# khiner/MeshEditor

Measured on AMD Instinct MI355X. Metric: eigenpairs/sec (K/M assembly + 50-mode solve, 100k-tet mesh), higher is better.
Workload: dtype f64; 1 GPU; cube_s100k: Kuhn mesh 105456 tets / 446631 DOF, NumModes=50 NumFemModes=65, P=10 excitation points, one mesh per GPU; eigenpairs_per_mesh=65, kept_modes_per_mesh=50, parallelism=mesh-per-gpu x1

## Files before the change

mesheditor_amd/csrc/mh_api.hip:

```cpp
#include "mh_common.h"

#include <algorithm>
#include <cmath>
#include <memory>

namespace {
constexpr int TB = 256;

__global__ void k_export_blocks(const uint32_t *__restrict__ row_ptr, const uint32_t *__restrict__ col, const uint32_t *__restrict__ perm, uint32_t nnodes,
                                uint32_t *__restrict__ row_out, uint32_t *__restrict__ col_out) {
    const uint32_t r = blockIdx.x * blockDim.x + threadIdx.x;
    if (r >= nnodes) return;
    for (uint32_t p = row_ptr[r]; p < row_ptr[r + 1]; ++p) {
        row_out[p] = perm[r];
        col_out[p] = perm[col[p]];
    }
}
__global__ void k_ref_to_panel(const double *__restrict__ xref, const uint32_t *__restrict__ perm, uint32_t nnodes, uint32_t w, double *__restrict__ panel) {
    const size_t i = size_t(blockIdx.x) * blockDim.x + threadIdx.x;
    if (i >= size_t(nnodes) * 3 * w) return;
    const uint32_t c = uint32_t(i % w), comp = uint32_t((i / w) % 3), node = uint32_t(i / (size_t(3) * w));
    panel[i] = xref[size_t(c) * (size_t(3) * nnodes) + size_t(3) * perm[node] + comp];
}
template<typename S, typename D> __global__ void k_cast(const S *__restrict__ src, D *__restrict__ dst, size_t count) {
// ... 97 lines not shown
            size_t free_bytes = 0, total_bytes = 0;
            if (hipMemGetInfo(&free_bytes, &total_bytes) != hipSuccess) total_bytes = 0, (void)hipGetLastError();
            ctx->pool.set_cap_for_device(total_bytes);
        }
        HIP_CHECK(hipStreamCreateWithFlags(&ctx->stream, hipStreamNonBlocking));
        ROCBLAS_CHECK(rocblas_create_handle(&ctx->blas));
        ROCBLAS_CHECK(rocblas_set_stream(ctx->blas, ctx->stream));
        ROCBLAS_CHECK(rocblas_set_pointer_mode(ctx->blas, rocblas_pointer_mode_host));
        ROCBLAS_CHECK(rocblas_set_atomics_mode(ctx->blas, rocblas_atomics_not_allowed));
        *out = ctx;
        return MH_OK;
    } catch (const std::exception &e) {
        const int code = mh_guard(ctx, e);
        fprintf(stderr, "modalhip: %s\n", e.what());
        if (ctx->blas) rocblas_destroy_handle(ctx->blas);
        if (ctx->blas_aux) rocblas_destroy_handle(ctx->blas_aux);
        if (ctx->aux_stream) (void)hipStreamDestroy(ctx->aux_stream);
        if (ctx->aux2_stream) (void)hipStreamDestroy(ctx->aux2_stream);
        for (hipEvent_t ev : ctx->ahead_ev) (void)hipEventDestroy(ev);
        if (ctx->stream) (void)hipStreamDestroy(ctx->stream);
        delete ctx;
        return code;
    }
}
void mh_context_destroy(mh_context *ctx) {
    if (!ctx) return;
    (void)hipSetDevice(ctx->device);
    (void)hipStreamSynchronize(ctx->stream);
    if (ctx->blas) rocblas_destroy_handle(ctx->blas);
    if (ctx->blas_aux) rocblas_destroy_handle(ctx->blas_aux);
    if (ctx->aux_stream) (void)hipStreamDestroy(ctx->aux_stream);
    if (ctx->aux2_stream) (void)hipStreamDestroy(ctx->aux2_stream);
    for (hipEvent_t e : ctx->ahead_ev) (void)hipEventDestroy(e);
    if (ctx->stream) (void)hipStreamDestroy(ctx->stream);
    delete ctx;
}
const char *mh_last_error(const mh_context *ctx) { return ctx ? ctx->last_error.c_str() : "null context"; }
int mh_context_synchronize(mh_context *ctx) {
    if (!ctx) return MH_EINVAL;
    try {
        HIP_CHECK(hipStreamSynchronize(ctx->stream));
        return MH_OK;
    } catch (const std::exception &e) { return mh_guard(ctx, e); }
}
void *mh_context_stream(mh_context *ctx) { return ctx ? ctx->stream : nullptr; }
int mh_context_time_kernels(mh_context *ctx, int enable) {
    if (!ctx) return MH_EINVAL;
    try {
        mh_timer_flush(ctx);
        ctx->time_kernels = enable != 0;
        for (auto &t : ctx->totals) t = {};
        return MH_OK;
    } catch (const std::exception &e) { return mh_guard(ctx, e); }
}
int mh_context_kernel_class_stats(mh_context *ctx, int kernel_class, uint64_t *launches, double *total_ms, double *total_work) {
    if (!ctx || kernel_class < 0 || kernel_class >= MH_KERNEL_CLASSES) return MH_EINVAL;
    try {
        mh_timer_flush(ctx);
        const auto &t = ctx->totals[kernel_class];
        if (launches) *launches = t.launches;
        if (total_ms) *total_ms = t.ms;
        if (total_work) *total_work = t.work;
        return MH_OK;
    } catch (const std::exception &e) { return mh_guard(ctx, e); }
}
int mh_context_kernel_stats(mh_context *ctx, uint64_t *launches, double *total_ms, double *total_bytes) {
// ... 200 lines not shown
```

mesheditor_amd/csrc/mh_common.h:

```cpp
#pragma once
#include "../../include/modalhip.h"

#include <hip/hip_runtime.h>
#include <rocblas/rocblas.h>
#include <rocsolver/rocsolver.h>

#include <algorithm>
#include <cstdarg>
#include <cstdio>
#include <cstdlib>
#include <cstring>
#include <iterator>
#include <map>
#include <mutex>
#include <stdexcept>
#include <string>
#include <vector>

struct MhError : std::runtime_error {
    int code;
    MhError(int c, const std::string &m) : std::runtime_error(m), code(c) {}
};

[[noreturn]] inline void mh_throw(int code, const char *fmt, ...) {
// ... 206 lines not shown
            else if (rocblas_set_stream(blas_aux, aux_stream) != rocblas_status_success) {
                (void)rocblas_destroy_handle(blas_aux);
                blas_aux = nullptr;
            }
        }
        return aux_stream != nullptr && blas_aux != nullptr;
    }
    hipStream_t aux2_stream{nullptr};
    std::vector<hipEvent_t> ahead_ev;
    bool aux2_stream_ready(size_t events = 0) {
        if (!aux2_stream && hipStreamCreateWithFlags(&aux2_stream, hipStreamNonBlocking) != hipSuccess) aux2_stream = nullptr, (void)hipGetLastError();
        while (aux2_stream && ahead_ev.size() < events) {
            hipEvent_t e = nullptr;
            if (hipEventCreateWithFlags(&e, hipEventDisableTiming) != hipSuccess) { (void)hipGetLastError(); return false; }
            ahead_ev.push_back(e);
        }
        return aux2_stream != nullptr;
    }
    rocblas_handle blas{nullptr};
    rocblas_handle blas_aux{nullptr};
    DevicePool pool;
    std::string last_error;
    hipEvent_t ev0{nullptr}, ev1{nullptr};
    void *gram_ws{nullptr};
    size_t gram_ws_bytes{0};
    uint32_t *iota{nullptr};
    unsigned long long *sytrd_xch{nullptr};
    uint32_t sytrd_epoch{0};
    int *sytrd_flag{nullptr};
    unsigned long long *sytrd_xch_wide{nullptr};
    uint32_t sytrd_epoch_wide{0};
    bool exchange_disabled{false};
    uint32_t sytrd_redos{0};
    unsigned long long *rr_check{nullptr};
    bool time_kernels{false};
    std::vector<std::pair<hipEvent_t, hipEvent_t>> timer_events;
    std::vector<double> timer_work;
    std::vector<int> timer_class;
    size_t timer_used{0};
    struct ClassTotals {
        double ms{0}, work{0};
        uint64_t launches{0};
    } totals[MH_KERNEL_CLASSES];
};
void mh_timer_flush(mh_context *ctx);
struct TimedLaunch {
    mh_context *ctx;
    bool on;
    size_t slot{0};
    TimedLaunch(mh_context *c, int kernel_class, double work) : ctx(c), on(c->time_kernels) {
        if (!on) return;
        if (ctx->timer_used == ctx->timer_events.size()) {
            hipEvent_t a, b;
            HIP_CHECK(hipEventCreate(&a));
            HIP_CHECK(hipEventCreate(&b));
            ctx->timer_events.emplace_back(a, b);
            ctx->timer_work.push_back(0);
            ctx->timer_class.push_back(0);
        }
        slot = ctx->timer_used++;
        ctx->timer_work[slot] = work;
        ctx->timer_class[slot] = kernel_class;
        HIP_CHECK(hipEventRecord(ctx->timer_events[slot].first, ctx->stream));
    }
    ~TimedLaunch() {
        if (on) (void)hipEventRecord(ctx->timer_events[slot].second, ctx->stream);
// ... 152 lines not shown
    } catch (const std::exception &e) {                \
        return mh_guard(ctx_guard_, e);                \
    }

inline unsigned div_up(size_t a, size_t b) { return unsigned((a + b - 1) / b); }

void mh_phase_shared_lock(int device);
void mh_phase_shared_unlock(int device);
struct MhSharedPhase {
    const int device;
    explicit MhSharedPhase(int dev) : device(dev) { mh_phase_shared_lock(device); }
    ~MhSharedPhase() { mh_phase_shared_unlock(device); }
    MhSharedPhase(const MhSharedPhase &) = delete;
    MhSharedPhase &operator=(const MhSharedPhase &) = delete;
};
std::mutex &mh_solve_mutex();
void mh_build_system(mh_context *ctx, const mh_mesh *mesh, const mh_material &mat, mh_system *sys);
void mh_build_hierarchy(mh_system *sys, double sigma, bool defer = false);
void mh_finish_hierarchy(mh_system *sys);
uint32_t mh_shift_invert_panel(mh_system *sys, double sigma, const double *b, double *x, uint32_t w, double rel_tol, uint32_t max_iters, double *worst_rel);
uint32_t mh_graph_aggregates(const std::vector<uint32_t> &row_ptr, const std::vector<uint32_t> &col, uint32_t n, uint32_t target, uint32_t max_order, std::vector<uint32_t> &agg_of);
void mh_select_patches(mh_system *sys, float threshold);
void mh_build_patch_inverses(mh_context *ctx, const BsrLevel &lvl, PatchSet &ps);
template<typename T>
void mh_apply_patches(mh_context *ctx, const PatchSet &ps, const T *in, const T *minus, uint32_t w, T coef, T *d, T *x, double *z, uint32_t wz, T *scratch);
void mh_gram(mh_context *ctx, size_t n, const double *x, uint32_t wa, const double *y, uint32_t wb, double *g, uint32_t ld, uint32_t ldy = 0, const uint32_t *ymap = nullptr);
void mh_combine(mh_context *ctx, size_t n, const double *x, uint32_t wx, const double *w, uint32_t ww, const double *p, uint32_t wp, const double *ct, uint32_t nc,
                double *out1, uint32_t n1, double *out2, bool accumulate = false, uint32_t ldx = 0, const uint32_t *xmap = nullptr, uint32_t ld1 = 0,
                const uint32_t *omap = nullptr, uint32_t col_begin = 0, uint32_t col_count = 0);
bool mh_tridiag_lowest_wide(mh_context *ctx, const double *d, const double *e, uint32_t m, uint32_t k, double *w, double *z, uint32_t ldz, double *work, int *info2,
                            double *quality_host);
void mh_apply_q(mh_context *ctx, const double *a, const double *tau, uint32_t m, double *z, uint32_t ldz, uint32_t ncols);
bool mh_tridiag_lowest(mh_context *ctx, const double *d, const double *e, uint32_t m, uint32_t k, double *w, double *z, uint32_t ldz, double *ufac,
                       double *quality, double *lam_scratch);
void mh_spd_inverse_small(mh_context *ctx, const double *a, uint32_t lda, uint32_t w, double *out, uint32_t ldo, int *info);
void mh_potrf(mh_context *ctx, double *a, uint32_t ld, uint32_t w, int *info);
void mh_potrf_small(mh_context *ctx, double *a, uint32_t w, int *info);
void mh_potrf_small_inverse(mh_context *ctx, double *a, uint32_t w, int *info, const double *dscale, double *linv);
bool mh_sytrd_gave_up(mh_context *ctx);
void mh_sytrd_wide(mh_context *ctx, double *a, uint32_t m, double *d, double *e, double *tau);
void mh_sytrd_small(mh_context *ctx, double *a, uint32_t m, double *d, double *e, double *tau, int variant = -1);
void mh_small_gemm(mh_context *ctx, bool ta, bool tb, uint32_t M, uint32_t N, uint32_t K, double alpha, const double *a, uint32_t lda, const double *b, uint32_t ldb, double beta, double *c,
                   uint32_t ldc);
void mh_short_product(mh_context *ctx, size_t n, const double *a, uint32_t m, const double *ct, uint32_t nc, double *out, double *partial, uint32_t slices);
void mh_pack_stacked(mh_context *ctx, const double *c1, uint32_t r1, const double *c2, uint32_t r2, uint32_t cols, double scale, double *ct);
void mh_pack_coefficients(mh_context *ctx, const double *c1, uint32_t n1, const double *c2, uint32_t n2, uint32_t m, uint32_t ld, double *ct);
void mh_spmm_mapped(mh_context *ctx, const BsrLevel &lvl, const double *vals9, const double *x, double *y, const double *mscal, double *y2, uint32_t w, uint32_t ldy,
                    uint32_t wreal, const uint32_t *omap, const double *res_theta = nullptr, double *res_out = nullptr, double *res_partial = nullptr,
                    const double *res_dinv = nullptr);
bool mh_spmm_f32_cheb_step(mh_context *ctx, const BsrLevel &lvl, const float *d_in, float *d_out, float *r, float *x, const float *dinv, float c1, float c2,
                           uint32_t w);
void mh_spmm_f32(mh_context *ctx, const BsrLevel &lvl, const float *x, float *y, uint32_t w);
void mh_spmm_mixed(mh_context *ctx, const BsrLevel &lvl, const float *x, double *y, uint32_t w);
const uint32_t *mh_identity_map(mh_context *ctx);
void mh_spmm(mh_context *ctx, const BsrLevel &lvl, const double *vals9, const double *x, double *y, const double *mscal, double *y2, uint32_t w);
```

mesheditor_amd/csrc/mh_dense.hip:

```cpp
#include "mh_common.h"

#include <optional>

#include <map>

struct PerDeviceOnce {
    static constexpr int MaxDevices = 64;
    std::once_flag flag[MaxDevices];
    template<typename F> void run(int device, F &&f) { std::call_once(flag[device >= 0 && device < MaxDevices ? device : 0], std::forward<F>(f)); }
};

static bool mh_test_own_gemm() {
    static const bool on = getenv("MH_TEST") && strstr(getenv("MH_TEST"), "own_gemm");
    return on;
}
namespace {
constexpr int KC = 32;

typedef double double4_t __attribute__((ext_vector_type(4)));

__host__ __device__ inline int pad_pitch(int w) {
    int p = ((w + 15) / 16) * 16;
    if ((p % 32) != 16) p += 16;
    return p;
// ... 1445 lines not shown
    for (int i = 0; i < m; ++i) X[size_t(i) * k + j] *= sc;
}
__global__ void __launch_bounds__(256) k_tridiag_residual(const double *__restrict__ D, const double *__restrict__ E, int m, const double *__restrict__ lam, const double *__restrict__ Z, int ldz,
                                                         unsigned long long *__restrict__ quality) {
    __shared__ double d[WIDE_T], e[WIDE_T], red[32], worst_of[4];
    const int tid = threadIdx.x, j = blockIdx.x;
    for (int i = tid; i < m; i += 256) d[i] = D[i], e[i] = i + 1 < m ? E[i] : 0.0;
    __syncthreads();
    double tnorm, pivmin;
    tridiag_scale(d, e, m, tid, 256, red, tnorm, pivmin);
    const double *z = Z + size_t(j) * ldz, lj = lam[j];
    double worst = 0.0;
    bool bad = false;
    for (int i = tid; i < m; i += 256) {
        const double r = (d[i] - lj) * z[i] + (i ? e[i - 1] * z[i - 1] : 0.0) + (i + 1 < m ? e[i] * z[i + 1] : 0.0);
        bad |= !(fabs(r) <= 1.7976931348623157e308);
        worst = fmax(worst, fabs(r));
    }
    if (bad) worst = __longlong_as_double(0x7ff8000000000000ll);
    for (int off = 32; off > 0; off >>= 1) {
        const double o = __shfl_xor(worst, off, 64);
        worst = (o != o || worst != worst) ? __longlong_as_double(0x7ff8000000000000ll) : fmax(worst, o);
    }
    if ((tid & 63) == 0) worst_of[tid >> 6] = worst;
    __syncthreads();
    if (tid == 0) {
        double q = 0.0;
        bool nan = false;
        for (int a = 0; a < 4; ++a) nan |= worst_of[a] != worst_of[a], q = fmax(q, worst_of[a]);
        q = nan ? __longlong_as_double(0x7ff8000000000000ll) : q / fmax(tnorm, 2.2250738585072014e-308);
        atomicMax(quality, static_cast<unsigned long long>(__double_as_longlong(q)));
    }
}
__global__ void __launch_bounds__(1024) k_tridiag_lowest(const double *__restrict__ D, const double *__restrict__ E, int m, int k, double *__restrict__ w,
                                                        double *__restrict__ z, int ldz, double *__restrict__ ufac, double *__restrict__ quality, const double *__restrict__ lam_in) {
    extern __shared__ __attribute__((aligned(16))) double sm[];
    double *d = sm, *e = d + 256, *e2 = e + 256, *lam = e2 + 256, *lo = lam + 256, *hi = lo + 256, *coef = hi + 256, *red = coef + 256;
    int *cnt = reinterpret_cast<int *>(red + 1024);
    double *X = red + 1024 + 512;
    const int tid = threadIdx.x, lane = tid & 63;
    if (tid < 256) {
        d[tid] = tid < m ? D[tid] : 0.0;
        const double ev = tid + 1 < m ? E[tid] : 0.0;
        e[tid] = ev;
        e2[tid] = ev * ev;
    }
    __syncthreads();
    {
        double gl = 1.7976931348623157e308, gh = -1.7976931348623157e308;
        for (int i = tid; i < m; i += 1024) {
            const double r = (i ? fabs(e[i - 1]) : 0.0) + fabs(e[i]);
            gl = fmin(gl, d[i] - r);
            gh = fmax(gh, d[i] + r);
        }
        for (int off = 32; off > 0; off >>= 1) {
            gl = fmin(gl, __shfl_xor(gl, off, 64));
            gh = fmax(gh, __shfl_xor(gh, off, 64));
        }
        if (lane == 0) { red[tid >> 6] = gl; red[16 + (tid >> 6)] = gh; }
    }
    __syncthreads();
    double glo = red[0], ghi = red[16];
    for (int q = 1; q < 16; ++q) { glo = fmin(glo, red[q]); ghi = fmax(ghi, red[16 + q]); }
    const double tnorm = fmax(fabs(glo), fabs(ghi));
    const double eps = 2.220446049250313e-16;
    double e2max = 0;
    for (int i = 0; i < m; ++i) e2max = fmax(e2max, e2[i]);
    const double pivmin = 2.2250738585072014e-308 * fmax(1.0, e2max);
// ... 156 lines not shown
            }
            __syncthreads();
            left = wave_sum_lds(red, m, lane);
            if (left > 0.5 || j == 0) break;
        }
        if ((tid >> 3) == j) my_inv2 = 1.0 / left;
        if (tid == 0) lo[j] = 1.0 / sqrt(left);
    }
    __syncthreads();
    for (int idx = tid; idx < m * k; idx += 1024) X[idx] *= lo[idx % k];
    __syncthreads();
    const long long t_gs = wall_clock64();
    double worst = 0;
    for (int idx = tid; idx < m * k; idx += 1024) {
        const int i = idx / k, j = idx % k;
        const double x = X[idx];
        const double r = (d[i] - lam[j]) * x + (i ? e[i - 1] * X[idx - k] : 0.0) + (i + 1 < m ? e[i] * X[idx + k] : 0.0);
        worst = fmax(worst, fabs(r));
        z[size_t(j) * ldz + i] = x;
    }
    for (int off = 32; off > 0; off >>= 1) worst = fmax(worst, __shfl_xor(worst, off, 64));
    __syncthreads();
    if (lane == 0) red[tid >> 6] = worst;
    __syncthreads();
    if (tid == 0) {
        double q = 0;
        for (int a = 0; a < 16; ++a) q = fmax(q, red[a]);
        *quality = q / fmax(tnorm, 2.2250738585072014e-308);
        quality[1] = double(t_bisect - t_start);
        quality[2] = double(t_invit - t_bisect);
        quality[3] = double(t_gs - t_invit);
        quality[4] = double(wall_clock64() - t_gs);
    }
    if (tid < k) w[tid] = lam[tid];
}
}

bool mh_tridiag_lowest(mh_context *ctx, const double *d, const double *e, uint32_t m, uint32_t k, double *w, double *z, uint32_t ldz, double *ufac, double *quality,
                       double *lam_scratch) {
    if (m < 2 || m > 256 || k < 1 || k > m || k > 128) return false;
    const size_t lds = (size_t(7) * 256 + 1024 + 512 + size_t(m) * k) * sizeof(double);
    if (lds > 158 * 1024) return false;
    static PerDeviceOnce attr;
    attr.run(ctx->device, [] { HIP_CHECK(hipFuncSetAttribute(reinterpret_cast<const void *>(&k_tridiag_lowest), hipFuncAttributeMaxDynamicSharedMemorySize, 160 * 1024)); });
    constexpr bool spread = true;
    if (spread) {
        k_tridiag_values<1><<<k, 256, 0, ctx->stream>>>(d, e, int(m), lam_scratch);
        KERNEL_CHECK();
    }
    k_tridiag_lowest<<<1, 1024, lds, ctx->stream>>>(d, e, int(m), int(k), w, z, int(ldz), ufac, quality, spread ? lam_scratch : nullptr);
    KERNEL_CHECK();
    return true;
}

bool mh_tridiag_lowest_wide(mh_context *ctx, const double *d, const double *e, uint32_t m, uint32_t k, double *w, double *z, uint32_t ldz, double *work, int *info2, double *quality_host) {
    if (m <= 256 || m > WIDE_T || k < 1 || k > 256 || k > m) return false;
    const size_t km = size_t(k) * m;
    double *xt = work, *xt2 = xt + km, *ufac = xt2 + km, *g = ufac + 3 * km, *linv = g + size_t(k) * k, *qual = linv + size_t(k) * k;
    k_tridiag_values<3><<<k, 256, 0, ctx->stream>>>(d, e, int(m), w);
    KERNEL_CHECK();
    k_tridiag_invit<<<div_up(k, 64), 64, 0, ctx->stream>>>(d, e, int(m), int(k), w, xt, ufac);
    KERNEL_CHECK();
    DevArray<int> info4_array(ctx, 4);
    int *info4 = info4_array.get();
    HIP_CHECK(hipMemsetAsync(info4, 0, 4 * sizeof(int), ctx->stream));
    for (int pass = 0; pass < 2; ++pass) {
        const double *src = pass == 0 ? xt : xt2;
        mh_small_gemm(ctx, false, true, k, k, m, 1.0, src, k, src, k, 0.0, g, k);
        mh_potrf(ctx, g, k, k, info4 + 2 * pass);
        HIP_CHECK(hipMemsetAsync(linv, 0, size_t(k) * k * sizeof(double), ctx->stream));
        ROCBLAS_CHECK(rocblas_dtrtri(ctx->blas, rocblas_fill_lower, rocblas_diagonal_non_unit, rocblas_int(k), g, rocblas_int(k), linv, rocblas_int(k)));
        if (pass == 0) mh_small_gemm(ctx, false, false, k, m, k, 1.0, linv, k, src, k, 0.0, xt2, k);
        else mh_small_gemm(ctx, true, true, m, k, k, 1.0, src, k, linv, k, 0.0, z, ldz);
    }
    HIP_CHECK(hipMemsetAsync(qual, 0, sizeof(double), ctx->stream));
    k_tridiag_residual<<<k, 256, 0, ctx->stream>>>(d, e, int(m), w, z, int(ldz), reinterpret_cast<unsigned long long *>(qual));
    KERNEL_CHECK();
    int hinfo[4] = {0, 0, 0, 0};
    HIP_CHECK(hipMemcpyAsync(quality_host, qual, sizeof(double), hipMemcpyDeviceToHost, ctx->stream));
    HIP_CHECK(hipMemcpyAsync(hinfo, info4, sizeof(hinfo), hipMemcpyDeviceToHost, ctx->stream));
    HIP_CHECK(hipStreamSynchronize(ctx->stream));
    if (hinfo[0] != 0 || hinfo[2] != 0) *quality_host = std::numeric_limits<double>::quiet_NaN();
    return true;
// ... 403 lines not shown
```

mesheditor_amd/csrc/mh_eigs.hip:

```cpp
#include "mh_common.h"

#include <algorithm>
#include <cmath>
#include <memory>
#include <condition_variable>
#include <mutex>
#include <numeric>
#include <optional>
#include <type_traits>

__global__ void k_shift_values(const double *kval, const double *mval, size_t nblocks, double sigma, double *aval);
__global__ void k_diag_inverse(const uint32_t *row_ptr, const uint32_t *col, const double *aval, uint32_t nnodes, double *dinv);
__global__ void k_coarse_matrix(const uint32_t *row_ptr, const uint32_t *col, const double *aval, const double *tmat, const uint32_t *agg_of, const uint32_t *agg_ptr,
                                const uint32_t *agg_nodes, uint32_t nagg, double *a0);
__global__ void k_fix_coarse_diag(double *a0, uint32_t n0, double rel);

namespace {
constexpr int TB = 256;

std::mutex g_solve_mutex;
struct Switches {
    bool verbose = getenv("MH_VERBOSE") != nullptr;
    bool fp32_prec = !(getenv("MH_PRECOND_FP64") && atoi(getenv("MH_PRECOND_FP64")) != 0);
    int deg2 = 0, deg1 = 0, gamma = 0;
    double cheb_ratio = 0.0, cheb_ratio1 = 0.0;
    bool test_sytrd_giveup = getenv("MH_TEST") && strstr(getenv("MH_TEST"), "sytrd_giveup");
    bool no_tridiag_wide = getenv("MH_TEST") && strstr(getenv("MH_TEST"), "no_tridiag_wide");
    bool test_last_resort = getenv("MH_TEST") && strstr(getenv("MH_TEST"), "last_resort");
    bool test_coarse_pivot = getenv("MH_TEST") && strstr(getenv("MH_TEST"), "coarse_pivot");
    bool test_selfcheck_fail = getenv("MH_TEST") && strstr(getenv("MH_TEST"), "selfcheck_fail");
    bool lmax_low = getenv("MH_TEST") && strstr(getenv("MH_TEST"), "lmax_low");
    bool potrf_chain = getenv("MH_TEST") && strstr(getenv("MH_TEST"), "potrf_chain");
    bool no_poly_start = getenv("MH_TEST") && strstr(getenv("MH_TEST"), "no_poly_start");
    Switches() {
        if (const char *c = getenv("MH_CYCLE")) {
            double v[5] = {0, 0, 0, 0, 0};
            sscanf(c, "%lf,%lf,%lf,%lf,%lf", &v[0], &v[1], &v[2], &v[3], &v[4]);
            deg2 = std::max(0, int(v[0])), deg1 = std::max(0, int(v[1])), gamma = std::max(0, int(v[2]));
            cheb_ratio = v[3];
            cheb_ratio1 = v[4];
        }
    }
};
const Switches &switches() {
    static const Switches s;
    return s;
}
constexpr int kPowerIterations = 20;
constexpr uint32_t kPrecondColumns = 256;
constexpr uint32_t kSkipP = 4;
constexpr uint32_t kGuardPercent = 10;
constexpr float kFlatShape = 1e-4f;
constexpr size_t kDenseLastResort = 12288;
constexpr int kLastResortCg = 8;

struct PhaseLock {
    std::mutex m;
    std::condition_variable cv;
    int readers = 0, writers_waiting = 0;
    bool writer = false;
    void lock_shared() {
        std::unique_lock<std::mutex> l(m);
        cv.wait(l, [&] { return !writer && writers_waiting == 0; });
        ++readers;
    }
    void unlock_shared() {
// ... 529 lines not shown
        rmax = fmax(rmax, fabs(r)), azmax = fmax(azmax, abs_az), zmax = fmax(zmax, fabs(zs[i]));
    }
    red[0][tid] = nan ? INFINITY : rmax, red[1][tid] = azmax, red[2][tid] = zmax;
    __syncthreads();
    for (int h = 128; h > 0; h >>= 1) {
        if (tid < uint32_t(h))
            for (int q = 0; q < 3; ++q) red[q][tid] = fmax(red[q][tid], red[q][tid + h]);
        __syncthreads();
    }
    if (tid == 0) {
        const double rel = red[0][0] / fmax(red[1][0] + fabs(th) * red[2][0], 1e-300);
        atomicMax(worst, (unsigned long long)__double_as_longlong(rel == rel ? rel : INFINITY));
    }
}
void rr_selfcheck(mh_context *ctx, const double *saved, uint32_t m, const double *z, uint32_t ldz, const double *theta, uint32_t ncols) {
    if (!ncols) return;
    if (!ctx->rr_check) {
        ctx->rr_check = static_cast<unsigned long long *>(ctx->pool.alloc(256));
        HIP_CHECK(hipMemsetAsync(ctx->rr_check, 0, 256, ctx->stream));
    }
    k_rr_selfcheck<<<3, 256, 0, ctx->stream>>>(saved, m, z, ldz, theta, ncols, ctx->rr_check);
    KERNEL_CHECK();
}

int host_info(DevArray<int> &info) { int hinfo = 0; info.download(&hinfo, 1); return hinfo; }
bool sytrd_gave_up(mh_context *ctx, int flag, double *gA, const double *saved, uint32_t m) {
    if (!flag && !switches().test_sytrd_giveup) return false;
    ++ctx->sytrd_redos;
    HIP_CHECK(hipMemcpyAsync(gA, saved, size_t(m) * m * sizeof(double), hipMemcpyDeviceToDevice, ctx->stream));
    return true;
}
bool accept_partial(mh_context *ctx, double quality, double *evals, const double *lam, uint32_t nwant) {
    if (!(quality < 1e-10)) return false;
    HIP_CHECK(hipMemcpyAsync(evals, lam, size_t(nwant) * sizeof(double), hipMemcpyDeviceToDevice, ctx->stream));
    return true;
}

int eig_tridiag_small(mh_context *ctx, double *gA, uint32_t m, double *evals, double *ework, DevArray<int> &info, uint32_t nwant, std::vector<double> *host_evals) {
    DevArray<double> z(ctx, size_t(m) * m), tau(ctx, m);
    const bool partial = nwant && nwant < m;
    DevArray<double> zl(ctx, partial ? size_t(m) * nwant : 0);
    double *zres = z.get();
    uint32_t ncols = m;
    HIP_CHECK(hipMemcpyAsync(z.get(), gA, size_t(m) * m * sizeof(double), hipMemcpyDeviceToDevice, ctx->stream));
    for (int attempt = 0; attempt < 2; ++attempt) {
        mh_sytrd_small(ctx, gA, m, evals, ework, tau, attempt == 0 ? -1 : 0);
        int gave_up = 0;
        const bool flagged = attempt == 0 && ctx->sytrd_flag;
        if (flagged) HIP_CHECK(hipMemcpyAsync(&gave_up, ctx->sytrd_flag, sizeof(int), hipMemcpyDeviceToHost, ctx->stream));
        if (partial) {
            DevArray<double> wv(ctx, 2 * m + 8), ufac(ctx, size_t(3) * m * nwant);
            double *zout = attempt == 0 ? zl.get() : z.get();
            if (mh_tridiag_lowest(ctx, evals, ework, m, nwant, wv, zout, m, ufac, wv.get() + m, wv.get() + m + 8)) {
                double qv[5] = {1, 0, 0, 0, 0};
                std::vector<double> lam_host(host_evals ? nwant : 0);
                HIP_CHECK(hipMemcpyAsync(qv, wv.get() + m, sizeof(qv), hipMemcpyDeviceToHost, ctx->stream));
                if (host_evals) HIP_CHECK(hipMemcpyAsync(lam_host.data(), wv.get(), size_t(nwant) * sizeof(double), hipMemcpyDeviceToHost, ctx->stream));
                HIP_CHECK(hipStreamSynchronize(ctx->stream));
                if (flagged && sytrd_gave_up(ctx, gave_up, gA, z, m)) continue;
                if (switches().verbose)
                    fprintf(stderr, "[rr] tridiagonal m %u lowest %u: residual / ||T|| %.2e; us: multisection %.0f, inverse iteration %.0f, Gram-Schmidt %.0f, output %.0f\n", m,
                            nwant, qv[0], qv[1] * 0.01, qv[2] * 0.01, qv[3] * 0.01, qv[4] * 0.01);
                if (accept_partial(ctx, qv[0], evals, wv, nwant)) {
                    if (host_evals) host_evals->swap(lam_host);
                    zres = zout, ncols = nwant;
                    break;
                }
            }
        }
        if (flagged) {
            HIP_CHECK(hipStreamSynchronize(ctx->stream));
            if (sytrd_gave_up(ctx, gave_up, gA, z, m)) continue;
        }
        ROCBLAS_CHECK(rocsolver_dstedc(ctx->blas, rocblas_evect_tridiagonal, m, evals, ework, z, m, info));
        if (const int hinfo = host_info(info)) return hinfo;
        break;
    }
    mh_apply_q(ctx, gA, tau, m, zres, m, ncols);
    if (zres == zl.get()) rr_selfcheck(ctx, z.get(), m, zres, m, evals, ncols);
    HIP_CHECK(hipMemcpyAsync(gA, zres, size_t(m) * ncols * sizeof(double), hipMemcpyDeviceToDevice, ctx->stream));
    return 0;
}

std::optional<int> eig_tridiag_wide(mh_context *ctx, double *gA, uint32_t m, double *evals, double *ework, DevArray<int> &info, uint32_t nwant) {
    DevArray<double> z(ctx, size_t(m) * m), saved(ctx, size_t(m) * m), tau(ctx, m);
    HIP_CHECK(hipMemcpyAsync(saved.get(), gA, size_t(m) * m * sizeof(double), hipMemcpyDeviceToDevice, ctx->stream));
    mh_sytrd_wide(ctx, gA, m, evals, ework, tau);
    int gave_up = 0;
    HIP_CHECK(hipMemcpyAsync(&gave_up, ctx->sytrd_flag, sizeof(int), hipMemcpyDeviceToHost, ctx->stream));
    HIP_CHECK(hipStreamSynchronize(ctx->stream));
    if (sytrd_gave_up(ctx, gave_up, gA, saved, m)) return std::nullopt;
    if (nwant && nwant < m && nwant <= 256 && !switches().no_tridiag_wide) {
        DevArray<double> work(ctx, size_t(5) * nwant * m + size_t(2) * nwant * nwant + 8), lam(ctx, nwant);
        double quality = 1.0;
        if (mh_tridiag_lowest_wide(ctx, evals, ework, m, nwant, lam, z, m, work, info, &quality)) {
            if (switches().verbose) fprintf(stderr, "[rr] tridiagonal m %u lowest %u (wide): residual / ||T|| %.2e\n", m, nwant, quality);
            if (accept_partial(ctx, quality, evals, lam, nwant)) {
                mh_apply_q(ctx, gA, tau, m, z, m, nwant);
                rr_selfcheck(ctx, saved.get(), m, z, m, evals, nwant);
                HIP_CHECK(hipMemcpyAsync(gA, z.get(), size_t(m) * nwant * sizeof(double), hipMemcpyDeviceToDevice, ctx->stream));
                HIP_CHECK(hipStreamSynchronize(ctx->stream));
                return 0;
            }
        }
    }
    ROCBLAS_CHECK(rocsolver_dstedc(ctx->blas, rocblas_evect_tridiagonal, m, evals, ework, z, m, info));
    if (const int hinfo = host_info(info)) return hinfo;
    ROCBLAS_CHECK(rocsolver_dormtr(ctx->blas, rocblas_side_left, rocblas_fill_lower, rocblas_operation_none, m, m, gA, m, tau, z, m));
    HIP_CHECK(hipMemcpyAsync(gA, z.get(), size_t(m) * m * sizeof(double), hipMemcpyDeviceToDevice, ctx->stream));
    HIP_CHECK(hipStreamSynchronize(ctx->stream));
    return 0;
// ... 515 lines not shown
            mh_spmm(ctx, sys->L2, sys->L2.aval, p, ap, nullptr, nullptr, w);
            dot(p, ap, pap, w);
            k_cg_advance<<<grid1(n * w), TB, 0, st>>>(z, rr, p, ap, rz, pap, n * w, w);
            KERNEL_CHECK();
            if (k + 1 == iters) break;
            prec.apply(rr, zz, w);
            dot(rr, zz, rz_new, w);
            k_cg_direction<<<grid1(n * w), TB, 0, st>>>(p, zz, rz_new, rz, n * w, w);
            KERNEL_CHECK();
            HIP_CHECK(hipMemcpyAsync(rz.get(), rz_new.get(), w * sizeof(double), hipMemcpyDeviceToDevice, st));
        }
    }
};
}

namespace {
struct BlockLobpcg {
    mh_system *sys;
    mh_context *ctx;
    hipStream_t st;
    const size_t n;
    const uint32_t nev, b, mmax;
    const double sigma, residual_tol;
    const uint32_t max_iters;
    const float *seed_basis;
    const uint32_t seed_rows, seed_cols;
    const volatile unsigned char *cancel;
    volatile float *progress;
    mh_profile &prof;
    mh_profile *profile;
    SharedPhase iterating;
    Timer t_iter;
    double precond_seconds = 0;
    double best_worst_active = 1e300;
    int floor_strikes = 0;
    std::vector<double> hist_active;
    uint32_t pairs_at_floor = 0;
    DevArray<double> X, AX, MX, Xn, AXn, MXn, W, AW, MW, P, MP, Pn, MPn, R, Rw;
    DevArray<double> gA, gM, gM0, gA0, App, evals, ework, Cp, T1, H, H2, G, dscale, Linv, theta_d, rn_d, mn_d, scratch, Ct, norms_d, theta_act_d, Hp, Up, Vp, T1p;
    DevArray<double> Linv_p, T1p2;
    DevArray<uint32_t> idx_d, pos_d;
    DevArray<double> Rr, res_partial, res_blocks, res_norms_d;
    std::vector<double> rr_evals;
    std::vector<uint32_t> res_act, res_pos;
    std::vector<double> res_norms;
    uint32_t res_pitch = 0;
    bool res_ready = false, rw_from_rr = false;
    DevArray<int> info;
    int inner_cg = 0;
    std::unique_ptr<Precond<float>> prec32;
    std::unique_ptr<Precond<double>> prec64;
    std::unique_ptr<PanelCg> panel_cg;
    const bool verbose = switches().verbose, fp32_prec = switches().fp32_prec;
    const bool pproj_ok;
    const bool scaled_norms;
    bool warm = false;
    bool w_implicit = false;
    int last_spread = 1 << 20;
    bool p_needs_explicit = false;
    uint32_t wp = 0;
    uint32_t iters = 0, nconv = 0, redos_at_start = 0;
    bool poly_allowed = true;
    std::vector<double> theta, rn, mn, xn, norms, theta_act, hist_worst;
    double anorm = 0;
    std::vector<uint32_t> act, order, hist_nconv;
    std::vector<uint8_t> locked;
// ... 301 lines not shown
                mh_throw(MH_ENOTCONVERGED, "LOBPCG: %u of %u pairs converged; the others sit at the rounding floor (residual %.1e and growing, best %.1e, tolerance %.1e)", nconv, nev,
                         worst_active, best_worst_active, residual_tol);
        }
        return false;
    }

    void search_directions(uint32_t it) {
        w = uint32_t(act.size());
        idx_d.upload(act.data(), w);
        const double *residuals = Rw.get();
        if (rw_from_rr) {
            if (act == res_act && res_pitch == w) {
                residuals = Rr.get();
            } else {
                std::vector<uint32_t> &pos = res_pos;
                pos.assign(w, 0);
                size_t q = 0;
                for (uint32_t k = 0; k < w; ++k) {
                    while (q < res_act.size() && res_act[q] != act[k]) ++q;
                    if (q == res_act.size()) mh_throw(MH_EHIP, "active column %u was not active before", act[k]);
                    pos[k] = uint32_t(q);
                }
                pos_d.upload(pos.data(), w);
                k_gather_cols<<<grid1(n * w), TB, 0, st>>>(Rr, pos_d, Rw, n, res_pitch, w);
                KERNEL_CHECK();
            }
        } else {
            k_gather_cols<<<grid1(n * w), TB, 0, st>>>(R, idx_d, Rw, n, b, w);
            KERNEL_CHECK();
        }
        for (uint32_t k = 0; k < w; ++k) theta_act[k] = theta[act[k]];
        theta_act_d.upload(theta_act.data(), w);
        {
            Timer tp(ctx);
            precondition(residuals, W, w);
            precond_seconds += tp.stop();
            prof.op_applications += w;
        }
        bool ok = true;
        p_implicit = false;
        if (pproj_ok && wp) {
            gram(ctx, n, MX, b, W, w, H, b);
            mh_pack_stacked(ctx, H, b, nullptr, 0, w, -1.0, Ct);
            mh_combine(ctx, n, X, b, nullptr, 0, nullptr, 0, Ct, w, W, w, nullptr, true);
            mh_spmm(ctx, sys->L2, sys->L2.aval, W, AW, sys->L2.mval, MW, w);
            gram(ctx, n, P, wp, MW, w, Hp, wp);
            lazy_images = true;
            w_implicit = false;
            ok = chol_orthonormalise(W, MW, AW, w, false, true, Hp, wp);
            if (!ok) mh_throw(MH_ENOTCONVERGED, "search directions lost rank at iteration %u", it);
            if (p_needs_explicit) {
                mh_pack_stacked(ctx, Hp, wp, nullptr, 0, w, -1.0, Ct);
                mh_combine(ctx, n, P, wp, nullptr, 0, nullptr, 0, Ct, w, W, w, nullptr, true);
                mh_spmm(ctx, sys->L2, sys->L2.aval, W, AW, sys->L2.mval, MW, w);
                lazy_images = w <= 256;
                ok = chol_orthonormalise(W, MW, AW, w, !lazy_images, lazy_images);
                if (!ok) mh_throw(MH_ENOTCONVERGED, "search directions lost rank at iteration %u", it);
            } else {
                p_implicit = true;
            }
        } else {
            gram(ctx, n, MX, b, W, w, H, b);
            if (wp) gram(ctx, n, MP, wp, W, w, H2, wp);
            mh_pack_stacked(ctx, H, b, H2, wp, w, -1.0, Ct);
            mh_combine(ctx, n, X, b, P, wp, nullptr, 0, Ct, w, W, w, nullptr, true);
            mh_spmm(ctx, sys->L2, sys->L2.aval, W, AW, sys->L2.mval, MW, w);
            lazy_images = w <= 256;
            w_implicit = false;
            ok = chol_orthonormalise(W, MW, AW, w, !lazy_images, lazy_images);
// ... 62 lines not shown
            k_symmetrize_lower<<<grid1(size_t(m) * m), TB, 0, st>>>(gA, m, m);
            KERNEL_CHECK();
            HIP_CHECK(hipMemcpyAsync(gA0, gA, size_t(m) * m * sizeof(double), hipMemcpyDeviceToDevice, st));
            HIP_CHECK(hipMemcpyAsync(gM0, gM, size_t(m) * m * sizeof(double), hipMemcpyDeviceToDevice, st));
            rr_evals.clear();
            const int hinfo = rr_solve(ctx, gA, gM, m, evals, ework, info, wa, gm_identity, &rr_evals);
            if (hinfo == 0) break;
            if (attempt == 1 || wp == 0) mh_throw(MH_ENOTCONVERGED, "Rayleigh-Ritz failed at iteration %u (info %d)", it, hinfo);
            wp = 0;
            m = wa + w;
        }
        if (rr_evals.size() == wa) std::copy(rr_evals.begin(), rr_evals.end(), theta_act.begin());
        else evals.download(theta_act.data(), wa);
        for (uint32_t k = 0; k < wa; ++k) theta[act[k]] = theta_act[k];
    }

    void conjugate_directions(uint32_t it) {
        const double one = 1, zero = 0, mone = -1;
        wp_new = w;
        k_build_cp<<<grid1(size_t(m) * w), TB, 0, st>>>(gA, nullptr, wa, m, w, m, Cp, m);
        KERNEL_CHECK();
        const double *mcp = gm_identity ? Cp.get() : T1.get();
        if (!gm_identity) ROCBLAS_CHECK(rocblas_dsymm(ctx->blas, rocblas_side_left, rocblas_fill_lower, m, w, &one, gM0, m, Cp, m, &zero, T1, m));
        small_dgemm(ctx, rocblas_operation_transpose, rocblas_operation_none, wa, w, m, &one, gA, m, mcp, m, &zero, H, wa);
        small_dgemm(ctx, rocblas_operation_none, rocblas_operation_none, m, w, wa, &mone, gA, m, H, wa, &one, Cp, m);
        if (!gm_identity) ROCBLAS_CHECK(rocblas_dsymm(ctx->blas, rocblas_side_left, rocblas_fill_lower, m, w, &one, gM0, m, Cp, m, &zero, T1, m));
        small_dgemm(ctx, rocblas_operation_transpose, rocblas_operation_none, w, w, m, &one, Cp, m, mcp, m, &zero, G, w);
        k_scale_gram<<<grid1(size_t(w) * w), TB, 0, st>>>(G, w, w, dscale);
        KERNEL_CHECK();
        {
            double *Gs = G.get() + size_t(w) * w;
            int hinfo = 0;
            const bool fused = w <= 128 && !switches().potrf_chain;
            {
                if (fused) mh_potrf_small_inverse(ctx, Gs, w, info, dscale, Linv_p);
                else mh_potrf(ctx, Gs, w, w, info);
                info.download(&hinfo, 1);
            }
            if (hinfo != 0) {
                wp_new = 0;
            } else if (fused) {
                mh_small_gemm(ctx, false, true, m, w, w, 1.0, Cp, m, Linv_p, w, 0.0, T1p2, m);
                HIP_CHECK(hipMemcpyAsync(Cp, T1p2, size_t(m) * w * sizeof(double), hipMemcpyDeviceToDevice, st));
            } else {
                k_unscale_chol<<<grid1(size_t(w) * w), TB, 0, st>>>(Gs, w, w, dscale);
                KERNEL_CHECK();
                ROCBLAS_CHECK(rocblas_dtrsm(ctx->blas, rocblas_side_right, rocblas_fill_lower, rocblas_operation_transpose, rocblas_diagonal_non_unit, m, w, &one, Gs, w, Cp, m));
            }
        }
        if (!warm && it < kSkipP && !hist_worst.empty() && hist_worst.back() > 0.5) wp_new = 0;
        if (wp_new) {
            small_dgemm(ctx, rocblas_operation_none, rocblas_operation_none, m, wp_new, m, &one, gA0, m, Cp, m, &zero, T1, m);
            small_dgemm(ctx, rocblas_operation_transpose, rocblas_operation_none, wp_new, wp_new, m, &one, Cp, m, T1, m, &zero, App, wp_new);
        }
    }

    void update_basis(uint32_t it) {
        mh_pack_coefficients(ctx, gA, wa, Cp, wp_new, m, m, Ct);
        {
            const uint32_t pitch = (wa + 1u) & ~1u;
            if (w_implicit) {
                const double unit = 1;
                double *rows = Ct.get() + size_t(wa) * (wa + wp_new);
                ROCBLAS_CHECK(rocblas_dtrmm(ctx->blas, rocblas_side_right, rocblas_fill_lower, rocblas_operation_none, rocblas_diagonal_non_unit, rocblas_int(wa + wp_new),
                                            rocblas_int(w), &unit, Linv, rocblas_int(w), rows, rocblas_int(wa + wp_new), rows, rocblas_int(wa + wp_new)));
            }
            if (p_implicit && wp) {
                const double minus = -1, plus = 1;
                const rocblas_int pitchc = rocblas_int(wa + wp_new);
                double *rows_w = Ct.get() + size_t(wa) * (wa + wp_new), *rows_p = Ct.get() + size_t(wa + w) * (wa + wp_new);
                ROCBLAS_CHECK(rocblas_dgemm(ctx->blas, rocblas_operation_none, rocblas_operation_transpose, pitchc, rocblas_int(wp), rocblas_int(w), &minus, rows_w, pitchc, Hp,
                                            rocblas_int(wp), &plus, rows_p, pitchc));
            }
            mh_combine(ctx, n, X, wa, W, w, P, wp, Ct, wa + wp_new, Xn, wa, Pn, false, b, idx_d, pitch);
            if (wp_new && !pproj_ok) mh_spmm(ctx, sys->L2, nullptr, Pn, nullptr, sys->L2.mval, MPn, wp_new);
            if (pitch == wa) k_scatter_cols<<<grid1(n * wa), TB, 0, st>>>(Xn.get(), idx_d, X.get(), n, b, wa);
            else k_scatter_cols_pitch<<<grid1(n * wa), TB, 0, st>>>(Xn.get(), pitch, idx_d, X.get(), n, b, wa);
            KERNEL_CHECK();
            if (Rr.count) {
                mh_spmm_mapped(ctx, sys->L2, sys->L2.aval, Xn, AX, sys->L2.mval, MX, pitch, b, wa, idx_d, evals, Rr, res_partial, scaled_norms ? sys->L2.dinv.get() : nullptr);
                const uint32_t rpb = 48, nblk = div_up(sys->n_nodes, rpb), w2 = 2 * pitch;
                dim3 grid(nblk, div_up(w2, 64));
                k_colsum_partial<<<grid, 64, 0, st>>>(res_partial, sys->n_nodes, w2, res_blocks, rpb);
                KERNEL_CHECK();
                k_colsumsq_final<<<w2, 256, 0, st>>>(res_blocks, nblk, w2, res_norms_d);
                KERNEL_CHECK();
                res_act = act;
                res_pitch = pitch;
                res_ready = true;
            } else {
                mh_spmm_mapped(ctx, sys->L2, sys->L2.aval, Xn, AX, sys->L2.mval, MX, pitch, b, wa, idx_d);
            }
        }
        std::swap(P, Pn); std::swap(MP, MPn);
        wp = wp_new;
    }

    void finish(double *eigenvalues) {
        prof.restarts = iters;
        prof.op_solve = precond_seconds;
        if (!converged) mh_throw(MH_ENOTCONVERGED, "LOBPCG: %u of %u pairs converged in %u iterations", nconv, nev, iters);
        for (uint32_t k = 0; k < nev; ++k) eigenvalues[k] = theta[order[k]] + sigma;
        sys->plain_residual = -1.0;
        if (scaled_norms) {
            theta_d.upload(theta.data(), b);
            const uint32_t rpb = 256, nblk = div_up(n, rpb);
            if (scratch.count < size_t(nblk) * 3 * b) scratch.reset(ctx, size_t(nblk) * 3 * b);
            k_residual_norms<<<dim3(nblk, div_up(b, 64)), 64, 0, st>>>(AX, MX, X, theta_d, 10.0 * std::abs(sigma), R, n, b, rpb, scratch, nullptr);
            KERNEL_CHECK();
            k_colsumsq_final<<<3 * b, 256, 0, st>>>(scratch, nblk, 3 * b, norms_d);
            KERNEL_CHECK();
            norms_d.download(norms.data(), 3 * size_t(b));
            double worst = 0;
            for (uint32_t k = 0; k < nev; ++k) {
                const uint32_t i = order[k];
                if (std::abs(theta[i]) < 10.0 * std::abs(sigma)) continue;
                worst = std::max(worst, std::sqrt(norms[i]) / (std::abs(theta[i]) * std::sqrt(norms[b + i])));
            }
            sys->plain_residual = worst;
            if (verbose) fprintf(stderr, "[lobpcg] accepted in the Jacobi-scaled norm at %.1e; worst elastic pair in the plain 2-norm: %.2e\n", residual_tol, worst);
        }
        sys->evecs.reset(ctx, n * nev);
        sys->evec_cols = nev;
        idx_d.upload(order.data(), nev);
        k_gather_cols<<<grid1(n * nev), TB, 0, st>>>(X, idx_d, sys->evecs, n, b, nev);
        KERNEL_CHECK();
        HIP_CHECK(hipStreamSynchronize(st));
        prof.iterate = t_iter.stop();
        read_health();
        sys->profile = prof;
        if (profile) *profile = prof;
        if (switches().test_selfcheck_fail && !ctx->exchange_disabled) prof.rr_selfcheck = 1.0;
// ... 244 lines not shown
```

Baseline: 613.2 eigenpairs/s.

## Overlap host readbacks with queued GPU work and drop per-iteration preconditioner sync

Small status readbacks (tridiagonal quality, eigenvalues, Cholesky info) now go through a reused pinned host buffer and an event. The host waits on that event only after queuing the follow-on work (apply_q, the C*Linv^T gemm), so the GPU keeps running instead of idling on a full stream synchronize. The preconditioner timer, which presumably synchronized every iteration, is replaced by recorded events that are summed in finish. The follow-on work is launched speculatively, which needs extra state (saving and restoring d, an applied flag). Creating two events per iteration adds some overhead.

Measured after the change: 618.9 eigenpairs/s (median of 6 runs). Within noise of the previous version (+0.9%).

```diff
diff --git a/mesheditor_amd/csrc/mh_api.hip b/mesheditor_amd/csrc/mh_api.hip
--- a/mesheditor_amd/csrc/mh_api.hip
+++ b/mesheditor_amd/csrc/mh_api.hip
@@ -153,6 +153,8 @@
     if (ctx->aux_stream) (void)hipStreamDestroy(ctx->aux_stream);
     if (ctx->aux2_stream) (void)hipStreamDestroy(ctx->aux2_stream);
     for (hipEvent_t e : ctx->ahead_ev) (void)hipEventDestroy(e);
+    if (ctx->back_ev) (void)hipEventDestroy(ctx->back_ev);
+    if (ctx->host_back) (void)hipHostFree(ctx->host_back);
     if (ctx->stream) (void)hipStreamDestroy(ctx->stream);
     delete ctx;
 }
diff --git a/mesheditor_amd/csrc/mh_common.h b/mesheditor_amd/csrc/mh_common.h
--- a/mesheditor_amd/csrc/mh_common.h
+++ b/mesheditor_amd/csrc/mh_common.h
@@ -262,6 +262,15 @@
     uint32_t sytrd_epoch_wide{0};
     bool exchange_disabled{false};
     uint32_t sytrd_redos{0};
+    double *host_back{nullptr};
+    hipEvent_t back_ev{nullptr};
+    double *host_back_ready() {
+        if (!host_back) {
+            HIP_CHECK(hipHostMalloc(reinterpret_cast<void **>(&host_back), 4096, hipHostMallocDefault));
+            HIP_CHECK(hipEventCreateWithFlags(&back_ev, hipEventDisableTiming));
+        }
+        return host_back;
+    }
     unsigned long long *rr_check{nullptr};
     bool time_kernels{false};
     std::vector<std::pair<hipEvent_t, hipEvent_t>> timer_events;
@@ -480,7 +489,7 @@
                             double *quality_host);
 void mh_apply_q(mh_context *ctx, const double *a, const double *tau, uint32_t m, double *z, uint32_t ldz, uint32_t ncols);
 bool mh_tridiag_lowest(mh_context *ctx, const double *d, const double *e, uint32_t m, uint32_t k, double *w, double *z, uint32_t ldz, double *ufac,
-                       double *quality, double *lam_scratch);
+                       double *quality, double *lam_scratch, double *d_save = nullptr);
 void mh_spd_inverse_small(mh_context *ctx, const double *a, uint32_t lda, uint32_t w, double *out, uint32_t ldo, int *info);
 void mh_potrf(mh_context *ctx, double *a, uint32_t ld, uint32_t w, int *info);
 void mh_potrf_small(mh_context *ctx, double *a, uint32_t w, int *info);
diff --git a/mesheditor_amd/csrc/mh_dense.hip b/mesheditor_amd/csrc/mh_dense.hip
--- a/mesheditor_amd/csrc/mh_dense.hip
+++ b/mesheditor_amd/csrc/mh_dense.hip
@@ -1501,8 +1501,8 @@
         atomicMax(quality, static_cast<unsigned long long>(__double_as_longlong(q)));
     }
 }
-__global__ void __launch_bounds__(1024) k_tridiag_lowest(const double *__restrict__ D, const double *__restrict__ E, int m, int k, double *__restrict__ w,
-                                                        double *__restrict__ z, int ldz, double *__restrict__ ufac, double *__restrict__ quality, const double *__restrict__ lam_in) {
+__global__ void __launch_bounds__(1024) k_tridiag_lowest(const double *D, const double *__restrict__ E, int m, int k, double *w, double *__restrict__ z, int ldz,
+                                                        double *__restrict__ ufac, double *__restrict__ quality, const double *__restrict__ lam_in, double *__restrict__ d_save) {
     extern __shared__ __attribute__((aligned(16))) double sm[];
     double *d = sm, *e = d + 256, *e2 = e + 256, *lam = e2 + 256, *lo = lam + 256, *hi = lo + 256, *coef = hi + 256, *red = coef + 256;
     int *cnt = reinterpret_cast<int *>(red + 1024);
@@ -1725,12 +1725,13 @@
         quality[3] = double(t_gs - t_invit);
         quality[4] = double(wall_clock64() - t_gs);
     }
+    if (d_save && tid < m) d_save[tid] = d[tid];
     if (tid < k) w[tid] = lam[tid];
 }
 }
 
 bool mh_tridiag_lowest(mh_context *ctx, const double *d, const double *e, uint32_t m, uint32_t k, double *w, double *z, uint32_t ldz, double *ufac, double *quality,
-                       double *lam_scratch) {
+                       double *lam_scratch, double *d_save) {
     if (m < 2 || m > 256 || k < 1 || k > m || k > 128) return false;
     const size_t lds = (size_t(7) * 256 + 1024 + 512 + size_t(m) * k) * sizeof(double);
     if (lds > 158 * 1024) return false;
@@ -1741,7 +1742,7 @@
         k_tridiag_values<1><<<k, 256, 0, ctx->stream>>>(d, e, int(m), lam_scratch);
         KERNEL_CHECK();
     }
-    k_tridiag_lowest<<<1, 1024, lds, ctx->stream>>>(d, e, int(m), int(k), w, z, int(ldz), ufac, quality, spread ? lam_scratch : nullptr);
+    k_tridiag_lowest<<<1, 1024, lds, ctx->stream>>>(d, e, int(m), int(k), w, z, int(ldz), ufac, quality, spread ? lam_scratch : nullptr, d_save);
     KERNEL_CHECK();
     return true;
 }
diff --git a/mesheditor_amd/csrc/mh_eigs.hip b/mesheditor_amd/csrc/mh_eigs.hip
--- a/mesheditor_amd/csrc/mh_eigs.hip
+++ b/mesheditor_amd/csrc/mh_eigs.hip
@@ -32,6 +32,7 @@
     bool lmax_low = getenv("MH_TEST") && strstr(getenv("MH_TEST"), "lmax_low");
     bool potrf_chain = getenv("MH_TEST") && strstr(getenv("MH_TEST"), "potrf_chain");
     bool no_poly_start = getenv("MH_TEST") && strstr(getenv("MH_TEST"), "no_poly_start");
+    bool partial_refused = getenv("MH_TEST") && strstr(getenv("MH_TEST"), "partial_refused");
     Switches() {
         if (const char *c = getenv("MH_CYCLE")) {
             double v[5] = {0, 0, 0, 0, 0};
@@ -627,7 +628,7 @@
 }
 bool accept_partial(mh_context *ctx, double quality, double *evals, const double *lam, uint32_t nwant) {
     if (!(quality < 1e-10)) return false;
-    HIP_CHECK(hipMemcpyAsync(evals, lam, size_t(nwant) * sizeof(double), hipMemcpyDeviceToDevice, ctx->stream));
+    if (lam != evals) HIP_CHECK(hipMemcpyAsync(evals, lam, size_t(nwant) * sizeof(double), hipMemcpyDeviceToDevice, ctx->stream));
     return true;
 }
 
@@ -637,6 +638,7 @@
     DevArray<double> zl(ctx, partial ? size_t(m) * nwant : 0);
     double *zres = z.get();
     uint32_t ncols = m;
+    bool applied = false;
     HIP_CHECK(hipMemcpyAsync(z.get(), gA, size_t(m) * m * sizeof(double), hipMemcpyDeviceToDevice, ctx->stream));
     for (int attempt = 0; attempt < 2; ++attempt) {
         mh_sytrd_small(ctx, gA, m, evals, ework, tau, attempt == 0 ? -1 : 0);
@@ -646,21 +648,27 @@
         if (partial) {
             DevArray<double> wv(ctx, 2 * m + 8), ufac(ctx, size_t(3) * m * nwant);
             double *zout = attempt == 0 ? zl.get() : z.get();
-            if (mh_tridiag_lowest(ctx, evals, ework, m, nwant, wv, zout, m, ufac, wv.get() + m, wv.get() + m + 8)) {
-                double qv[5] = {1, 0, 0, 0, 0};
-                std::vector<double> lam_host(host_evals ? nwant : 0);
-                HIP_CHECK(hipMemcpyAsync(qv, wv.get() + m, sizeof(qv), hipMemcpyDeviceToHost, ctx->stream));
-                if (host_evals) HIP_CHECK(hipMemcpyAsync(lam_host.data(), wv.get(), size_t(nwant) * sizeof(double), hipMemcpyDeviceToHost, ctx->stream));
-                HIP_CHECK(hipStreamSynchronize(ctx->stream));
+            if (mh_tridiag_lowest(ctx, evals, ework, m, nwant, evals, zout, m, ufac, wv.get() + m, wv.get() + m + 8, wv.get())) {
+                const size_t nback = 8 + (host_evals ? nwant : 0);
+                double *back = ctx->host_back_ready();
+                HIP_CHECK(hipMemcpyAsync(back, wv.get() + m, nback * sizeof(double), hipMemcpyDeviceToHost, ctx->stream));
+                HIP_CHECK(hipEventRecord(ctx->back_ev, ctx->stream));
+                applied = !flagged;
+                if (applied) mh_apply_q(ctx, gA, tau, m, zout, m, nwant);
+                HIP_CHECK(hipEventSynchronize(ctx->back_ev));
+                const double *qv = back;
+                const auto restore_d = [&] { HIP_CHECK(hipMemcpyAsync(evals, wv.get(), size_t(m) * sizeof(double), hipMemcpyDeviceToDevice, ctx->stream)); };
                 if (flagged && sytrd_gave_up(ctx, gave_up, gA, z, m)) continue;
                 if (switches().verbose)
                     fprintf(stderr, "[rr] tridiagonal m %u lowest %u: residual / ||T|| %.2e; us: multisection %.0f, inverse iteration %.0f, Gram-Schmidt %.0f, output %.0f\n", m,
                             nwant, qv[0], qv[1] * 0.01, qv[2] * 0.01, qv[3] * 0.01, qv[4] * 0.01);
-                if (accept_partial(ctx, qv[0], evals, wv, nwant)) {
-                    if (host_evals) host_evals->swap(lam_host);
+                if (!switches().partial_refused && accept_partial(ctx, qv[0], evals, evals, nwant)) {
+                    if (host_evals) host_evals->assign(back + 8, back + nback);
                     zres = zout, ncols = nwant;
                     break;
                 }
+                applied = false;
+                restore_d();
             }
         }
         if (flagged) {
@@ -671,7 +679,7 @@
         if (const int hinfo = host_info(info)) return hinfo;
         break;
     }
-    mh_apply_q(ctx, gA, tau, m, zres, m, ncols);
+    if (!applied) mh_apply_q(ctx, gA, tau, m, zres, m, ncols);
     if (zres == zl.get()) rr_selfcheck(ctx, z.get(), m, zres, m, evals, ncols);
     HIP_CHECK(hipMemcpyAsync(gA, zres, size_t(m) * ncols * sizeof(double), hipMemcpyDeviceToDevice, ctx->stream));
     return 0;
@@ -1253,6 +1261,7 @@
     SharedPhase iterating;
     Timer t_iter;
     double precond_seconds = 0;
+    std::vector<hipEvent_t> precond_marks;
     double best_worst_active = 1e300;
     int floor_strikes = 0;
     std::vector<double> hist_active;
@@ -1620,9 +1629,14 @@
         for (uint32_t k = 0; k < w; ++k) theta_act[k] = theta[act[k]];
         theta_act_d.upload(theta_act.data(), w);
         {
-            Timer tp(ctx);
+            hipEvent_t mark[2];
+            for (hipEvent_t &e : mark) {
+                HIP_CHECK(hipEventCreate(&e));
+                precond_marks.push_back(e);
+            }
+            HIP_CHECK(hipEventRecord(mark[0], st));
             precondition(residuals, W, w);
-            precond_seconds += tp.stop();
+            HIP_CHECK(hipEventRecord(mark[1], st));
             prof.op_applications += w;
         }
         bool ok = true;
@@ -1751,17 +1765,22 @@
             double *Gs = G.get() + size_t(w) * w;
             int hinfo = 0;
             const bool fused = w <= 128 && !switches().potrf_chain;
-            {
-                if (fused) mh_potrf_small_inverse(ctx, Gs, w, info, dscale, Linv_p);
-                else mh_potrf(ctx, Gs, w, w, info);
+            if (fused) {
+                mh_potrf_small_inverse(ctx, Gs, w, info, dscale, Linv_p);
+                double *back = ctx->host_back_ready();
+                HIP_CHECK(hipMemcpyAsync(back, info.get(), sizeof(int), hipMemcpyDeviceToHost, st));
+                HIP_CHECK(hipEventRecord(ctx->back_ev, st));
+                mh_small_gemm(ctx, false, true, m, w, w, 1.0, Cp, m, Linv_p, w, 0.0, T1p2, m);
+                HIP_CHECK(hipMemcpyAsync(Cp, T1p2, size_t(m) * w * sizeof(double), hipMemcpyDeviceToDevice, st));
+                HIP_CHECK(hipEventSynchronize(ctx->back_ev));
+                memcpy(&hinfo, back, sizeof(int));
+            } else {
+                mh_potrf(ctx, Gs, w, w, info);
                 info.download(&hinfo, 1);
             }
             if (hinfo != 0) {
                 wp_new = 0;
-            } else if (fused) {
-                mh_small_gemm(ctx, false, true, m, w, w, 1.0, Cp, m, Linv_p, w, 0.0, T1p2, m);
-                HIP_CHECK(hipMemcpyAsync(Cp, T1p2, size_t(m) * w * sizeof(double), hipMemcpyDeviceToDevice, st));
-            } else {
+            } else if (!fused) {
                 k_unscale_chol<<<grid1(size_t(w) * w), TB, 0, st>>>(Gs, w, w, dscale);
                 KERNEL_CHECK();
                 ROCBLAS_CHECK(rocblas_dtrsm(ctx->blas, rocblas_side_right, rocblas_fill_lower, rocblas_operation_transpose, rocblas_diagonal_non_unit, m, w, &one, Gs, w, Cp, m));
@@ -1815,8 +1834,21 @@
         wp = wp_new;
     }
 
+    void release_marks() {
+        for (hipEvent_t e : precond_marks) (void)hipEventDestroy(e);
+        precond_marks.clear();
+    }
+    ~BlockLobpcg() { release_marks(); }
+
     void finish(double *eigenvalues) {
         prof.restarts = iters;
+        for (size_t k = 0; k + 1 < precond_marks.size(); k += 2) {
+            float ms = 0;
+            HIP_CHECK(hipEventSynchronize(precond_marks[k + 1]));
+            HIP_CHECK(hipEventElapsedTime(&ms, precond_marks[k], precond_marks[k + 1]));
+            precond_seconds += ms * 1e-3;
+        }
+        release_marks();
         prof.op_solve = precond_seconds;
         if (!converged) mh_throw(MH_ENOTCONVERGED, "LOBPCG: %u of %u pairs converged in %u iterations", nconv, nev, iters);
         for (uint32_t k = 0; k < nev; ++k) eigenvalues[k] = theta[order[k]] + sigma;
```
